# HoangChuongNguyen/ibgs

Hardware: AMD Instinct MI355X
Metric: train-step fps (fwd+bwd raster) @1080p, 1M Gaussians (higher is better)
Workload: dtype f32

## Files before the change

ibgs_amd/csrc/binning.hip:

```cpp
#include "common.h"
#include "wave_bits.h"

namespace ibgs {

constexpr int CB = BIN_CELL;
constexpr int XCHUNK = BIN_XCHUNK;

struct RectU { uint32_t x0, x1, y0, y1; };
struct Footprint { RectU r; uint64_t m0, m1, m2, m3; bool masked, rows; };
static_assert(IBGS_CULL_WORDS == 4, "four mask words");
__device__ __forceinline__ Footprint make_footprint(const uint4 rr, const uint64_t* __restrict__ tmask_hi, uint32_t id)
{
    Footprint f;
    f.r = RectU{rr.x & 0xFFFFu, rr.x >> 16, rr.y & 0xFFFFu, rr.y >> 16};
    const uint32_t area = (f.r.x1 - f.r.x0) * (f.r.y1 - f.r.y0);
    f.masked = area <= (uint32_t)IBGS_CULL_MAX_TILES;
    f.m0 = ((uint64_t)rr.w << 32) | rr.z;
    f.rows = !f.masked && f.m0 == 0ull;
    const uint64_t* mw = tmask_hi + (size_t)id * (IBGS_CULL_WORDS - 1);
    f.m1 = (f.masked && area > 64u) ? mw[0] : 0ull;
    f.m2 = (f.masked && area > 128u) ? mw[1] : 0ull;
    f.m3 = (f.masked && area > 192u) ? mw[2] : 0ull;
    return f;
}
// ... 464 lines not shown
            s_base[c] += (uint32_t)(__popcll(s_touch[c]) + __popcll(s_touch[nc + c]) + __popcll(s_touch[2 * nc + c]) + __popcll(s_touch[3 * nc + c]));
        __syncthreads();
    }
}

__device__ __forceinline__ int cell_of_chunk(const uint32_t* __restrict__ cell_chunk0, int ncells, uint32_t ch)
{
    int lo = 0, hi = ncells;
    while (hi - lo > 1) { const int mid = (lo + hi) >> 1; if (cell_chunk0[mid] <= ch) lo = mid; else hi = mid; }
    return lo;
}

__global__ void __launch_bounds__(64) expand_count_kernel(const uint32_t* __restrict__ cell_start, const uint32_t* __restrict__ cell_chunk0, int ncells,
                                                          const uint4* __restrict__ cent,
                                                          uint32_t* __restrict__ chunk_cnt )
{
    const uint32_t ch = blockIdx.x;
    if (ch >= cell_chunk0[ncells]) return;
    const int lane = threadIdx.x;
    const int cell = cell_of_chunk(cell_chunk0, ncells, ch);
    const uint32_t i0 = cell_start[cell] + (ch - cell_chunk0[cell]) * XCHUNK, i1 = min(cell_start[cell + 1], i0 + XCHUNK);
    uint32_t mlo[XCHUNK / 64], mhi[XCHUNK / 64];
#pragma unroll
    for (int rd = 0; rd < XCHUNK / 64; rd++) {
        const uint32_t i = i0 + (uint32_t)rd * 64 + lane;
        const uint4 e = (i < i1) ? cent[i] : make_uint4(0u, 0u, 0u, 0u);
        mlo[rd] = e.z; mhi[rd] = e.w;
    }
    const BitTransposeConsts btc = bit_transpose_consts(lane);
    uint32_t cnt = 0;
#pragma unroll
    for (int rd = 0; rd < XCHUNK / 64; rd++) {
        if (i0 + (uint32_t)rd * 64 >= i1) break;
        wave_bit_transpose64(mlo[rd], mhi[rd], btc);
        cnt += (uint32_t)__popc(mlo[rd]) + (uint32_t)__popc(mhi[rd]);
    }
    chunk_cnt[(size_t)ch * 64 + lane] = cnt;
}

constexpr int TR_WAVES = 16;
__global__ void __launch_bounds__(64 * TR_WAVES) tile_ranges_kernel(int ntiles, uint32_t* __restrict__ tile_start ,
                                                                   uint32_t* __restrict__ ranges, uint32_t* __restrict__ counters , uint32_t cap,
                                                                   const uint32_t* __restrict__ sort_flag ,
                                                                   uint32_t* __restrict__ host_note , uint32_t note_ticket)
{
    constexpr int NW = TR_WAVES;
    __shared__ uint32_t s_wave[NW];
    const int tid = threadIdx.x, lane = tid & 63, wave = tid >> 6;
    const int per_wave = ((ntiles + NW - 1) / NW + 63) / 64 * 64;
    const int w0 = min(ntiles, wave * per_wave), w1 = min(ntiles, w0 + per_wave);
    constexpr int KEEP = 32;
    const int nsteps = (w1 - w0 + 63) / 64;
    uint32_t v[KEEP];
    uint32_t sum = 0;
#pragma unroll
    for (int k = 0; k < KEEP; k++) { const int t = w0 + k * 64 + lane; v[k] = (k < nsteps && t < w1) ? tile_start[t] : 0u; sum += v[k]; }
    for (int k = KEEP; k < nsteps; k++) { const int t = w0 + k * 64 + lane; sum += t < w1 ? tile_start[t] : 0u; }
#pragma unroll
    for (int d = 32; d >= 1; d >>= 1) sum += (uint32_t)__shfl_xor((int)sum, d, 64);
    if (lane == 0) s_wave[wave] = sum;
    __syncthreads();
    uint32_t run = 0;
    for (int w = 0; w < wave; w++) run += s_wave[w];
    auto step = [&](int k, uint32_t n) {
        uint32_t inc = n;
#pragma unroll
        for (int d = 1; d < 64; d <<= 1) { const uint32_t o = (uint32_t)__shfl_up((int)inc, d, 64); if (lane >= d) inc += o; }
        const uint32_t start = run + inc - n;
        const int t = w0 + k * 64 + lane;
        if (t < w1) {
            tile_start[t] = start;
            const uint32_t a = min(start, cap), b = min(start + n, cap);
            *reinterpret_cast<uint2*>(ranges + 2 * (size_t)t) = (b > a) ? make_uint2(a, b) : make_uint2(0u, 0u);
        }
        run += (uint32_t)__shfl((int)inc, 63, 64);
    };
#pragma unroll
    for (int k = 0; k < KEEP; k++) if (k < nsteps) step(k, v[k]);
    for (int k = KEEP; k < nsteps; k++) { const int t = w0 + k * 64 + lane; step(k, t < w1 ? tile_start[t] : 0u); }
    if (tid == NW * 64 - 1) {
        tile_start[ntiles] = run; counters[0] = run;
        if (host_note) {
            host_note[0] = run; host_note[2] = counters[2]; if (sort_flag && *sort_flag) host_note[3] = 1u;
            __threadfence_system();
            __hip_atomic_store(host_note + 4, note_ticket, __ATOMIC_RELEASE, __HIP_MEMORY_SCOPE_SYSTEM);
        }
    }
}

constexpr int CSCAN_WAVES = 8;
__global__ void __launch_bounds__(64 * CSCAN_WAVES) cell_scan_kernel(const uint32_t* __restrict__ cell_chunk0, int ncells, int cgx, int gx, int gy,
                                                                     uint32_t* __restrict__ chunk_cnt, uint32_t* __restrict__ tile_total )
{
    __shared__ uint32_t s_sum[CSCAN_WAVES][64];
    const int cell = blockIdx.x, lane = threadIdx.x & 63, wave = threadIdx.x >> 6;
    const uint32_t c0 = cell_chunk0[cell], c1 = cell_chunk0[cell + 1];
    const uint32_t per = (c1 - c0 + CSCAN_WAVES - 1) / CSCAN_WAVES;
    const uint32_t w0 = min(c1, c0 + (uint32_t)wave * per), w1 = min(c1, w0 + per);
    uint32_t sum = 0;
    for (uint32_t ch = w0; ch < w1; ch += 8) {
        uint32_t c[8];
#pragma unroll
        for (int k = 0; k < 8; k++) c[k] = (ch + k < w1) ? chunk_cnt[(size_t)(ch + k) * 64 + lane] : 0u;
#pragma unroll
        for (int k = 0; k < 8; k++) sum += c[k];
    }
    s_sum[wave][lane] = sum;
    __syncthreads();
    uint32_t run = 0, total = 0;
#pragma unroll
    for (int w = 0; w < CSCAN_WAVES; w++) { const uint32_t v = s_sum[w][lane]; if (w < wave) run += v; total += v; }
    for (uint32_t ch = w0; ch < w1; ch += 8) {
        uint32_t c[8];
#pragma unroll
        for (int k = 0; k < 8; k++) c[k] = (ch + k < w1) ? chunk_cnt[(size_t)(ch + k) * 64 + lane] : 0u;
#pragma unroll
        for (int k = 0; k < 8; k++) if (ch + k < w1) { chunk_cnt[(size_t)(ch + k) * 64 + lane] = run; run += c[k]; }
    }
    const int tx = (cell % cgx) * CB + (lane & 7), ty = (cell / cgx) * CB + (lane >> 3);
    if (wave == 0 && tx < gx && ty < gy) tile_total[ty * gx + tx] = total;
}

constexpr int SCAT_STAGE = 4096;
__global__ void __launch_bounds__(64) expand_scatter_kernel(const uint32_t* __restrict__ cell_start, const uint32_t* __restrict__ cell_chunk0, int ncells,
                                                            int cgx, int gx, int gy, const uint4* __restrict__ cent,
                                                            const uint32_t* __restrict__ chunk_pref, const uint32_t* __restrict__ tile_start,
                                                            uint32_t cap, uint32_t* __restrict__ point_list)
{
    __shared__ uint32_t s_id[XCHUNK / 64][64];
    __shared__ uint8_t s_out[SCAT_STAGE];
    const uint32_t ch = blockIdx.x;
    if (ch >= cell_chunk0[ncells]) return;
    const int lane = threadIdx.x;
    const int cell = cell_of_chunk(cell_chunk0, ncells, ch);
    const uint32_t i0 = cell_start[cell] + (ch - cell_chunk0[cell]) * XCHUNK, i1 = min(cell_start[cell + 1], i0 + XCHUNK);
    const int tx = (cell % cgx) * CB + (lane & 7), ty = (cell / cgx) * CB + (lane >> 3);
    const uint32_t slot0 = (tx < gx && ty < gy) ? tile_start[ty * gx + tx] + chunk_pref[(size_t)ch * 64 + lane] : 0u;
    uint32_t mlo[XCHUNK / 64], mhi[XCHUNK / 64];
#pragma unroll
    for (int rd = 0; rd < XCHUNK / 64; rd++) {
        const uint32_t i = i0 + (uint32_t)rd * 64 + lane;
        const uint4 e = (i < i1) ? cent[i] : make_uint4(0u, 0u, 0u, 0u);
        mlo[rd] = e.z; mhi[rd] = e.w;
        s_id[rd][lane] = e.x;
    }
    const BitTransposeConsts btc = bit_transpose_consts(lane);
    uint32_t n = 0;
#pragma unroll
    for (int rd = 0; rd < XCHUNK / 64; rd++) {
        if (i0 + (uint32_t)rd * 64 < i1) wave_bit_transpose64(mlo[rd], mhi[rd], btc);
        n += (uint32_t)__popc(mlo[rd]) + (uint32_t)__popc(mhi[rd]);
    }
    uint32_t inc = n;
#pragma unroll
    for (int d = 1; d < 64; d <<= 1) { const uint32_t o = (uint32_t)__shfl_up((int)inc, d, 64); if (lane >= d) inc += o; }
    const uint32_t total = (uint32_t)__builtin_amdgcn_readlane((int)inc, 63);
    const bool staged = total <= (uint32_t)SCAT_STAGE;
    const uint32_t base = inc - n;
    __syncthreads();
    uint32_t k = staged ? base : slot0;
#pragma unroll
    for (int rd = 0; rd < XCHUNK / 64; rd++) {
#pragma unroll
        for (int half = 0; half < 2; half++) {
            uint32_t bits = half ? mhi[rd] : mlo[rd];
            while (bits != 0u) {
                const int l = __builtin_ctz(bits) + 32 * half;
                bits &= bits - 1u;
// ... 87 lines not shown
```

ibgs_amd/csrc/render_bwd.hip:

```cpp
#include "common.h"
#include <stdlib.h>
#include "wave_reduce.h"
#include <type_traits>

namespace ibgs {

struct BwdParams {
    const uint32_t* ranges; const uint32_t* point_list; const float4* rec;
    Cam cam;
    int ntiles;
    TileMap tmap;
    int n_src; int tex_quant;
    int power_skip;
    const uint32_t* tile_risky;
    const float* ref_to_src; const float4* src_rgba;
    const float* final_T; const uint32_t* n_contrib; const float* sum_w; const uint32_t* low_high;
    const int32_t* valid_idx; const float* valid_w;
    const float* depth_pixels; const float* warped_pixels;
    const float* dL_dcolor; const float* dL_dnormal; const float* dL_ddepth; const float* dL_dwarped;
    float* gacc;
    int tab_slots;
    const uint32_t* slot_c; const uint32_t* meta; float* tab;
    const uint32_t* order;
    int slab_ipt;
// ... 643 lines not shown
                        const float S0 = Q[0] + Q[1];
                        const float t = dx0 * S0;
                        v[0] = fmaf(-8.0f, Q[1], t); v[1] = dy0 * S0;
                        v[4] = fmaf(dx0, fmaf(-16.0f, Q[1], t), 64.0f * Q[1]);
                        v[5] = dy0 * v[0]; v[6] = dy0 * v[1];
                        v[7] = S0;
                    } else {
                        const float qdx = Q[0] * dx0, qdy = Q[0] * dy0;
                        v[0] = qdx; v[1] = qdy; v[4] = qdx * dx0; v[5] = qdx * dy0; v[6] = qdy * dy0; v[7] = Q[0];
                    }
                    v[2] = aX; v[3] = aY;
                    v[8] = vR; v[9] = vG; v[10] = vB; v[11] = vNx; v[12] = vNy; v[13] = vNz; v[14] = vD; v[15] = 0.f;
                    const float tot = wave_transpose_reduce16(v, lane);
                    const uint32_t id = __float_as_uint(q0.w);
                    if (col >= 0) {
                        if (p.slab) p.slab[((size_t)(r0 + k) * (p.slab_ipt ? p.slab_ipt : IPT) + (size_t)sub) * GACC_FLOATS + col] = tot;
                        else atomicAdd(p.gacc + (size_t)id * GACC_FLOATS + col, tot);
                    }
                }
            }
        };
        if (bg0) { if (stable) chunk(std::true_type{}, std::true_type{}); else chunk(std::false_type{}, std::true_type{}); }
        else { if (stable) chunk(std::true_type{}, std::false_type{}); else chunk(std::false_type{}, std::false_type{}); }
        __syncthreads();
        top -= count;
    }
}

#ifdef IBGS_TRACE_WAVES
__device__ uint4 g_trace_bwd[IBGS_TRACE_MAX];
#endif
__global__ void __launch_bounds__(64, 8) render_bwd_color_kernel(BwdParams p)
{
    IBGS_TRACE_BEGIN();
    int tile, sub = 0;
    bool have;
    if (p.order) { const uint32_t t = p.order[blockIdx.x]; tile = (int)(t & ~ORDER_SPLIT_BIT); have = t != 0xFFFFFFFFu; }
    else have = tile_map_item(p.tmap, blockIdx.x, p.cam.gx, p.cam.gy, 1, tile, sub);
    __shared__ float4 s_rec[3][BWD_CHUNK];
    __shared__ __align__(16) unsigned char s_pix[4 * WAVE * sizeof(float4)];
    if (have && !tile_is_risky(p.tile_risky, tile)) render_bwd_color_body<4, true, false, true>(p, tile, sub, s_rec, reinterpret_cast<float4 (*)[WAVE]>(s_pix));
    IBGS_TRACE_END(g_trace_bwd);
}
__global__ void __launch_bounds__(64, 8) render_bwd_color_noabs_kernel(BwdParams p)
{
    int tile, sub = 0;
    bool have;
    if (p.order) { const uint32_t t = p.order[blockIdx.x]; tile = (int)(t & ~ORDER_SPLIT_BIT); have = t != 0xFFFFFFFFu; }
    else have = tile_map_item(p.tmap, blockIdx.x, p.cam.gx, p.cam.gy, 1, tile, sub);
    __shared__ float4 s_rec[3][BWD_CHUNK];
    __shared__ __align__(16) unsigned char s_pix[4 * WAVE * sizeof(float4)];
    if (have && !tile_is_risky(p.tile_risky, tile)) render_bwd_color_body<4, false, false, true>(p, tile, sub, s_rec, reinterpret_cast<float4 (*)[WAVE]>(s_pix));
}
template <bool ABS>
__global__ void __launch_bounds__(64, 4) render_bwd_color_risk_kernel(BwdParams p)
{
    __shared__ float4 s_rec[3][BWD_CHUNK];
    __shared__ float4 s_gpix[4][WAVE];
    int tile = (int)blockIdx.x;
    if (p.order) { const uint32_t t = p.order[blockIdx.x]; if (t == 0xFFFFFFFFu) return; tile = (int)(t & ~ORDER_SPLIT_BIT); }
    if (tile >= p.ntiles || !tile_is_risky(p.tile_risky, tile)) return;
    render_bwd_color_body<4, ABS, true>(p, tile, 0, s_rec, s_gpix);
}

constexpr int ORDER_SNAKE_ROUNDS = 8;
__global__ void __launch_bounds__(1024) tile_order_kernel(int ntiles, int nslots , int slot_rounds ,
                                                          const uint32_t* __restrict__ walked_waves, const uint32_t* __restrict__ meta, uint32_t* __restrict__ order,
                                                          uint32_t* __restrict__ order_out ,
                                                          int theta_pct = 0 )
{
    __shared__ uint32_t s_hist[1024];
    __shared__ uint32_t s_w[16];
    __shared__ uint32_t s_max;
    __shared__ unsigned long long s_total;
    const int tid = threadIdx.x, lane = tid & 63, wave = tid >> 6;
    const uint32_t ipt = meta[10];
    if (ipt != 1u && ipt != 2u && ipt != 4u) {
        for (int i = tid; i < nslots; i += 1024) { const uint32_t v = i < ntiles ? ((uint32_t)i | (theta_pct > 0 ? ORDER_SPLIT_BIT : 0u)) : 0xFFFFFFFFu; order[i] = v; if (order_out) order_out[i] = v; }
        return;
    }
    auto walked_of = [&](int t) { uint32_t v = walked_waves[(size_t)t * ipt]; for (uint32_t k = 1; k < ipt; k++) v = max(v, walked_waves[(size_t)t * ipt + k]); return v; };
    s_hist[tid] = 0u;
    if (tid == 0) { s_max = 0u; s_total = 0ull; }
    for (int i = tid; i < nslots; i += 1024) { order[i] = 0xFFFFFFFFu; if (order_out) order_out[i] = 0xFFFFFFFFu; }
    __syncthreads();
    constexpr int KEEP = 16;
    uint32_t w[KEEP];
    uint32_t m = 0;
    unsigned long long sum = 0ull;
#pragma unroll
    for (int k = 0; k < KEEP; k++) { const int t = tid + k * 1024; w[k] = t < ntiles ? walked_of(t) : 0u; m = max(m, w[k]); sum += w[k]; }
    for (int t = tid + KEEP * 1024; t < ntiles; t += 1024) { const uint32_t v = walked_of(t); m = max(m, v); sum += v; }
    for (int d = 32; d >= 1; d >>= 1) m = max(m, (uint32_t)__shfl_xor((int)m, d, 64));
    if (lane == 0) atomicMax(&s_max, m);
    if (theta_pct > 0) {
        for (int d = 32; d >= 1; d >>= 1) sum += __shfl_xor(sum, d, 64);
        if (lane == 0) atomicAdd(&s_total, sum);
    }
    __syncthreads();
    const uint32_t mx = s_max;
    const unsigned long long total = s_total;
    const int sh = mx >= 1024u ? (32 - __builtin_clz(mx)) - 10 : 0;
    auto bucket = [&](uint32_t v) { return 1023u - min(v >> sh, 1023u); };
#pragma unroll
    for (int k = 0; k < KEEP; k++) if (tid + k * 1024 < ntiles) atomicAdd(&s_hist[bucket(w[k])], 1u);
    for (int t = tid + KEEP * 1024; t < ntiles; t += 1024) atomicAdd(&s_hist[bucket(walked_of(t))], 1u);
    __syncthreads();
    const uint32_t v = s_hist[tid];
    uint32_t inc = v;
    for (int d = 1; d < 64; d <<= 1) { const uint32_t o = (uint32_t)__shfl_up((int)inc, d, 64); if (lane >= d) inc += o; }
    if (lane == 63) s_w[wave] = inc;
    __syncthreads();
    uint32_t before = 0;
    for (int ww = 0; ww < wave; ww++) before += s_w[ww];
    s_hist[tid] = before + inc - v;
    __syncthreads();
    const uint32_t nrounds = (uint32_t)nslots / (uint32_t)ORDER_CLASSES;
    auto put = [&](int t, uint32_t key) {
        const uint32_t r = atomicAdd(&s_hist[bucket(key)], 1u);
        const uint32_t stratum = r / ORDER_CLASSES, c = r % ORDER_CLASSES;
        uint32_t slot = r;
        if (nrounds <= (uint32_t)slot_rounds) {
            const uint32_t round = (stratum + 1u) % nrounds;
            slot = round * ORDER_CLASSES + ((stratum & 1u) ? ORDER_CLASSES - 1u - c : c);
        }
        const uint32_t word = (uint32_t)t | ((theta_pct > 0 && hybrid_split(key, total, (uint32_t)theta_pct)) ? ORDER_SPLIT_BIT : 0u);
        order[slot] = word;
        if (order_out) order_out[slot] = word;
    };
#pragma unroll
    for (int k = 0; k < KEEP; k++) if (tid + k * 1024 < ntiles) put(tid + k * 1024, w[k]);
    for (int t = tid + KEEP * 1024; t < ntiles; t += 1024) put(t, walked_of(t));
}
__global__ void __launch_bounds__(64, 8) render_bwd_color_small_kernel(BwdParams p)
{
    int tile, sub;
    __shared__ float4 s_rec[3][BWD_CHUNK];
    __shared__ float4 s_gpix[1][WAVE];
    if (tile_map_item(p.tmap, blockIdx.x, p.cam.gx, p.cam.gy, 4, tile, sub) && !tile_is_risky(p.tile_risky, tile)) render_bwd_color_body<1>(p, tile, sub, s_rec, s_gpix);
}
template <bool ABS>
__global__ void __launch_bounds__(64, 8) render_bwd_color_hybrid_kernel(BwdParams p)
{
    __shared__ float4 s_rec[3][BWD_CHUNK];
    __shared__ float4 s_gpix[4][WAVE];
    int tile, sub; bool split;
    if (!hybrid_item(blockIdx.x, p.hybrid_grid1, p.order, tile, sub, split) || tile_is_risky(p.tile_risky, tile)) return;
    if (split) render_bwd_color_body<1, ABS>(p, tile, sub, s_rec, s_gpix);
    else if (sub == 0) render_bwd_color_body<4, ABS>(p, tile, 0, s_rec, s_gpix);
}
template <int PPL, bool ABS>
__device__ __forceinline__ void render_bwd_geo_entry(const BwdParams& p)
{
    __shared__ float4 s_rec[4][BWD_CHUNK];
    __shared__ float4 s_gpix[PPL][WAVE];
    __shared__ float4 s_gnrm[PPL][WAVE];
    int tile, sub;
    if (PPL == 4 && p.order) { const uint32_t t = p.order[blockIdx.x]; if (t == 0xFFFFFFFFu) return; tile = (int)(t & ~ORDER_SPLIT_BIT); sub = 0; }
    else if (!tile_map_item(p.tmap, blockIdx.x, p.cam.gx, p.cam.gy, 4 / PPL, tile, sub)) return;
    if (tile_is_risky(p.tile_risky, tile)) return;
    render_bwd_geo_body<PPL, ABS>(p, tile, sub, s_rec, s_gpix, s_gnrm);
}
template <bool ABS>
__global__ void __launch_bounds__(64, 3) render_bwd_geo_risk_kernel(BwdParams p)
{
    __shared__ float4 s_rec[4][BWD_CHUNK];
    __shared__ float4 s_gpix[4][WAVE];
    __shared__ float4 s_gnrm[4][WAVE];
    int tile = (int)blockIdx.x;
    if (p.order) { const uint32_t t = p.order[blockIdx.x]; if (t == 0xFFFFFFFFu) return; tile = (int)(t & ~ORDER_SPLIT_BIT); }
    if (tile >= p.ntiles || !tile_is_risky(p.tile_risky, tile)) return;
    render_bwd_geo_body<4, ABS, true>(p, tile, 0, s_rec, s_gpix, s_gnrm);
}
__global__ void __launch_bounds__(64, 4) render_bwd_geo4_kernel(BwdParams p) { render_bwd_geo_entry<4, true>(p); }
__global__ void __launch_bounds__(64, 4) render_bwd_geo4_noabs_kernel(BwdParams p) { render_bwd_geo_entry<4, false>(p); }
__global__ void __launch_bounds__(64, 6) render_bwd_geo_kernel(BwdParams p) { render_bwd_geo_entry<1, true>(p); }
template <bool ABS>
__global__ void __launch_bounds__(64, 4) render_bwd_geo_hybrid_kernel(BwdParams p)
{
    __shared__ float4 s_rec[4][BWD_CHUNK];
    __shared__ float4 s_gpix[4][WAVE];
    __shared__ float4 s_gnrm[4][WAVE];
    int tile, sub; bool split;
    if (!hybrid_item(blockIdx.x, p.hybrid_grid1, p.order, tile, sub, split) || tile_is_risky(p.tile_risky, tile)) return;
    if (split) render_bwd_geo_body<1, ABS>(p, tile, sub, s_rec, s_gpix, s_gnrm);
    else if (sub == 0) render_bwd_geo_body<4, ABS>(p, tile, 0, s_rec, s_gpix, s_gnrm);
}

int render_backward_ref_arith(uint32_t flags)
{
    if (flags & IBGS_FLAG_NO_REF_POWER_SKIP) return 0;
    return RA_DECIDE | ((flags & IBGS_FLAG_REF_ARITH) ? RA_ASSOC : RA_LFORM);
}

int render_backward_waves_per_tile(const ibgs_backward_args& a)
{
    const int nt = ((a.W + TILE - 1) / TILE) * ((a.H + TILE - 1) / TILE);
    if (a.render_geo) return ((a.flags & IBGS_FLAG_QUADRANT_WAVES) ? false : ((a.flags & IBGS_FLAG_TILE_WAVES) ? true : nt >= 4096)) ? 1 : 4;
    return ((a.flags & IBGS_FLAG_QUADRANT_WAVES) ? true : ((a.flags & IBGS_FLAG_TILE_WAVES) ? false : nt < hybrid_max_tiles())) ? 4 : 1;
}

int launch_render_backward(hipStream_t s, const ibgs_backward_args& a, const GeomState& g, const BinState& b,
                           const ImgState& im, const float4* src_rgba, float* slab, float* geo_tab)
{
    BwdParams p;
    p.ranges = im.ranges; p.point_list = b.point_list; p.rec = reinterpret_cast<const float4*>(g.rec);
    p.cam = make_cam(a.viewmatrix, a.projmatrix, a.campos, a.bg, a.tanfovx, a.tanfovy, a.W, a.H);
    p.ntiles = p.cam.gx * p.cam.gy;
// ... 105 lines not shown
```

ibgs_amd/csrc/render_fwd.hip:

```cpp
#include "common.h"

namespace ibgs {

struct FwdParams {
    const uint32_t* ranges; const uint32_t* point_list; const float4* rec;
    Cam cam;
    int ntiles;
    TileMap tmap;
    int n_views, gyv; float fxv[IBGS_MAX_VIEWS], fyv[IBGS_MAX_VIEWS];
    int n_src; int L; float thr; int tex_quant;
    int power_skip;
    const float* ref_to_src; const float* src_cam_pos; const float4* src_rgba; const float* src_depths;
    int ds0, ds1, ds2, ds3, ds4;
    float* final_T; uint32_t* n_contrib; float* sum_w; uint32_t* low_high; int32_t* valid_idx; float* valid_w; uint32_t* slot_c; uint32_t* meta; uint32_t* walked;
    uint32_t* risky;
    int hybrid_grid1;
    int hybrid;
    const uint32_t* order;
    float* out_color; float* out_normal; float* out_depth; float* out_cam_feat; float* out_warped;
    float* out_min_depth_diff; float* out_camera_ray; int32_t* out_mask;
};

enum { MODE_COLOR = 0, MODE_GEO = 1, MODE_DEPTH = 2 };

// ... 86 lines not shown
#pragma unroll
    for (int q = 0; q < PPL; q++) {
        const int qq = quad0 + q;
        px[q] = tx0 + (qq & 1) * 8 + (lane & 7);
        py[q] = ty0 + (qq >> 1) * 8 + (lane >> 3);
        pxf[q] = (float)px[q]; pyf[q] = (float)py[q];
        inside[q] = px[q] < W && py[q] < H;
        live[q] = __builtin_amdgcn_ballot_w64(inside[q]);
        recm[q] = live[q];
        T[q] = 1.0f; C[q][0] = C[q][1] = C[q][2] = 0.f; lastc[q] = 0;
    }
    const float pxf_t0 = (float)(tx0 + (lane & 7)), pyf_t0 = (float)(ty0 + (lane >> 3));
    const float fx = (DEPTH && p.n_views > 1) ? p.fxv[view] : p.cam.fx, fy = (DEPTH && p.n_views > 1) ? p.fyv[view] : p.cam.fy;
    const float cx = (float)(W * 0.5f), cy = (float)(H * 0.5f);
    const float eps = 1.0e-8f;

    float Nacc[PPL][3];
    constexpr bool RING_LDS = GEO && PPL <= 2;
    __shared__ float s_bw[RING_LDS ? PPL : 1][RING_LDS ? MAXL : 1][RING_LDS ? WAVE : 1];
    __shared__ uint32_t s_bc[RING_LDS ? PPL : 1][RING_LDS ? MAXL : 1][RING_LDS ? WAVE : 1];
    float bd[PPL][RING_LDS ? 1 : MAXL], bw[PPL][RING_LDS ? 1 : MAXL]; uint32_t bc[PPL][RING_LDS ? 1 : MAXL];
    int before_ptr[PPL], below_count[PPL];
    float tot_w[PPL], wd_sum[PPL];
    int resume[PPL]; uint32_t cnt[PPL];
    float rayx[PPL], rayy[PPL];
    const int L = p.L;
    if (GEO && blockIdx.x == 0 && lane == 0) p.meta[0] = (uint32_t)L;
    const int before_cap = (L % 2 == 0) ? (L / 2) : ((L + 1) / 2);
    const int below_cap = L - before_cap;
    if (GEO || DEPTH) {
#pragma unroll
        for (int q = 0; q < PPL; q++) {
            Nacc[q][0] = Nacc[q][1] = Nacc[q][2] = 0.f;
#pragma unroll
            for (int s = 0; s < MAXL; s++) {
                if (RING_LDS) { s_bw[q][s][lane] = 0.f; s_bc[q][s][lane] = 0u; }
                else if (s < (RING_LDS ? 1 : MAXL)) { bd[q][s] = 0.f; bw[q][s] = 0.f; bc[q][s] = 0u; }
            }
            before_ptr[q] = 0; below_count[q] = 0; tot_w[q] = 0.f; wd_sum[q] = 0.f; resume[q] = 0; cnt[q] = 0;
            rayx[q] = (pxf[q] - cx) / fx; rayy[q] = (pyf[q] - cy) / fy;
        }
    }

    const uint32_t r0 = p.ranges[2 * tile], r1 = p.ranges[2 * tile + 1];
    const int n = (int)(r1 - r0);

    auto fetch_quad = [&](int base) -> float4 {
        const int e = base + (lane >> 2);
        if (e < n) return p.rec[(size_t)p.point_list[r0 + e] * 4 + (lane & 3)];
        return make_float4(0.f, 0.f, 0.f, 0.f);
    };
    float4 ahead = make_float4(0.f, 0.f, 0.f, 0.f);
    if constexpr (GEO) ahead = fetch_quad(0);
    int base = 0;
    uint64_t riskany = 0ull;
    for (; base < n; base += CHUNK) {
        uint64_t riskm = 0ull;
        if constexpr (GEO) {
            float4 v = ahead;
            const int qd = lane & 3;
            const bool risky = qd == 1 && base + (lane >> 2) < n && conic_takes_ref_power(v.x, v.y, v.z);
            if (qd == 0) v.z = -__builtin_amdgcn_logf(v.z);
            if (qd == 1) { v.x *= EXP2_SCALE; v.y *= EXP2_SCALE; v.z *= EXP2_SCALE; }
            s_rec[qd][lane >> 2] = v;
            if (p.power_skip) riskm = __builtin_amdgcn_ballot_w64(risky);
            ahead = fetch_quad(base + CHUNK);
        } else {
            const int e = base + lane;
            bool risky = false;
            if (e < n) {
                const uint32_t id = p.point_list[r0 + e];
                const float4* r = p.rec + (size_t)id * 4;
                float4 c0 = r[0], c1 = r[1];
                risky = conic_takes_ref_power(c1.x, c1.y, c1.z);
                stage_for_exp2(c0, c1);
                s_rec[0][lane] = c0;
                s_rec[1][lane] = c1;
                s_rec[2][lane] = DEPTH ? r[3] : r[2];
            }
            if (p.power_skip) riskm = __builtin_amdgcn_ballot_w64(risky);
        }
        riskany |= riskm;
        __syncthreads();
        const int count = min(CHUNK, n - base);
        for (int j = 0; j < count; j++) {
            const float4 q0 = s_rec[0][j];
            const float4 q1 = s_rec[1][j];
            const float4 q2 = s_rec[2][j];
            float4 q3 = q2;
            if constexpr (GEO) q3 = s_rec[3][j];
            const int e = base + j;
            IBGS_LANES_ADD(0, 1);
#ifdef IBGS_COUNT_LANES
            bool lc_any_ = false;
#endif
            uint32_t e1v = (uint32_t)(e + 1);
            asm volatile("" : "+v"(e1v));
            const float dx0 = q0.x - (TILE_Q >= 0 ? pxf_t0 : pxf[0]), dy0 = q0.y - (TILE_Q >= 0 ? pyf_t0 : pyf[0]);
            const float lx0 = q1.x * dx0 + q1.y * dy0, ly0 = q1.y * dx0 + q1.z * dy0;
            const float P0 = fmaf(dx0, lx0, fmaf(dy0, ly0, q0.z));
            float p2q[PPL];
            p2q[0] = P0;
            if (PPL >= 2) p2q[1] = fmaf(-16.0f, lx0, P0 + 64.0f * q1.x);
            if (PPL == 4) {
                p2q[2] = fmaf(-16.0f, ly0, P0 + 64.0f * q1.z);
                p2q[3] = fmaf(128.0f, q1.y, p2q[2] + (p2q[1] - P0));
            }
            if constexpr (TILE_Q >= 1 && PPL == 1) {
                const float E1 = fmaf(-16.0f, lx0, P0 + 64.0f * q1.x);
                const float E2 = fmaf(-16.0f, ly0, P0 + 64.0f * q1.z);
                p2q[0] = TILE_Q == 1 ? E1 : (TILE_Q == 2 ? E2 : fmaf(128.0f, q1.y, E2 + (E1 - P0)));
            }
            if ((riskm >> (GEO ? 4 * j + 1 : j)) & 1ull) {
                const uint32_t gid = p.point_list[r0 + e];
                const float4 g0 = p.rec[(size_t)gid * 4], g1 = p.rec[(size_t)gid * 4 + 1];
#pragma unroll
                for (int q = 0; q < PPL; q++) p2q[q] = ref_power_E(g0.x - pxf[q], g0.y - pyf[q], g1.x, g1.y, g1.z, q0.z);
            }
#pragma unroll
            for (int q = 0; q < PPL; q++) {
                if (live[q] == 0ull) continue;
                const float p2 = p2q[q];
                uint64_t m = __builtin_amdgcn_ballot_w64(p2 <= ALPHA_SKIP_E) & live[q];
                if (DEPTH) {
                    const uint64_t running = __builtin_amdgcn_ballot_w64(e >= resume[q]) & live[q];
                    if (__builtin_amdgcn_inverse_ballot_w64(running)) cnt[q]++;
                    m &= running;
                }
                if (m == 0ull) continue;
                IBGS_LANES_ADD(2, 64); IBGS_LANES_ADD(3, __builtin_popcountll(m));
#ifdef IBGS_COUNT_LANES
                lc_any_ = true;
#endif
                const float alpha = fminf(0.99f, __builtin_amdgcn_exp2f(-p2));
                const float aeff = __builtin_amdgcn_inverse_ballot_w64(m) ? alpha : 0.f;
                float aT = aeff * T[q];
                float test_T = T[q] - aT;
                const uint64_t fin = __builtin_amdgcn_ballot_w64(test_T < 0.0001f) & m;
                if (fin != 0ull) {
                    const bool pf = __builtin_amdgcn_inverse_ballot_w64(fin);
                    aT = pf ? 0.f : aT;
                    test_T = pf ? T[q] : test_T;
                    live[q] &= ~fin;
                    m &= ~fin;
                }
                const bool acc = __builtin_amdgcn_inverse_ballot_w64(m);
                const uint32_t contributor = DEPTH ? cnt[q] : e1v;
                if (!DEPTH) { C[q][0] += q2.x * aT; C[q][1] += q2.y * aT; C[q][2] += q2.z * aT; }
                if (GEO) { Nacc[q][0] += q3.x * aT; Nacc[q][1] += q3.y * aT; Nacc[q][2] += q3.z * aT; }
                if ((GEO && (m & recm[q]) != 0ull) || DEPTH) {
                    const float denom = q3.x * rayx[q] + q3.y * rayy[q] + q3.z + eps;
                    float dep = 0.f;
                    if (DEPTH) dep = -q1.w / denom;
                    const bool pos = DEPTH ? (dep > 0.0f) : (q1.w * denom < 0.0f);
                    const bool hit = acc && pos;
                    const bool front = T[q] > 0.5f;
                    int slot = -1;
                    if (hit && front) slot = before_ptr[q];
                    else if (hit && below_count[q] < below_cap) slot = before_cap + below_count[q];
                    if (DEPTH && slot >= 0 && front) {
                        float oldw = 0.f, oldd = 0.f;
#pragma unroll
                        for (int s = 0; s < (RING_LDS ? 1 : MAXL); s++) if (s == slot) { oldw = bw[q][s]; oldd = bd[q][s]; }
                        tot_w[q] -= oldw; wd_sum[q] -= oldw * oldd;
                    }
                    if (slot >= 0) {
                        if (RING_LDS) { s_bw[q][slot][lane] = aT; s_bc[q][slot][lane] = contributor; }
                        else {
#pragma unroll
                            for (int s = 0; s < (RING_LDS ? 1 : MAXL); s++) if (s == slot) { if (DEPTH) bd[q][s] = dep; bw[q][s] = aT; bc[q][s] = contributor; }
                        }
                        if (front) { const int nb = before_ptr[q] + 1; before_ptr[q] = (nb == before_cap) ? 0 : nb; }
                        else below_count[q]++;
                        if (DEPTH) { tot_w[q] += aT; wd_sum[q] += aT * dep; }
                    }
                    if (DEPTH && hit && below_count[q] == below_cap) {
                        resume[q] = (e / 256 + 1) * 256;
                    }
                    if (DEPTH && below_cap > 0) {
                        live[q] &= ~__builtin_amdgcn_ballot_w64(hit && below_count[q] == below_cap);
                    }
                    if (GEO) recm[q] &= ~__builtin_amdgcn_ballot_w64(test_T <= 0.5f && below_count[q] >= below_cap);
                }
                T[q] = test_T;
                lastc[q] = acc ? contributor : lastc[q];
            }
#ifdef IBGS_COUNT_LANES
            if (lc_any_) IBGS_LANES_ADD(1, 1);
#endif
        }
        __syncthreads();
        uint64_t anylive = 0ull;
#pragma unroll
        for (int q = 0; q < PPL; q++) anylive |= live[q];
        if (anylive == 0ull) break;
    }

#pragma unroll
    for (int q = 0; q < PPL; q++) {
        if (!inside[q]) continue;
        const size_t pix = vbase + (size_t)py[q] * W + px[q];
        p.final_T[pix] = T[q];
        p.n_contrib[pix] = lastc[q];
        if (!DEPTH) {
            p.out_color[pix] = C[q][0] + T[q] * p.cam.bg[0];
            p.out_color[HW + pix] = C[q][1] + T[q] * p.cam.bg[1];
            p.out_color[2 * HW + pix] = C[q][2] + T[q] * p.cam.bg[2];
        }
        if (DEPTH) p.out_depth[pix] = wd_sum[q] / (tot_w[q] + eps);
        if (GEO) { p.out_normal[pix] = Nacc[q][0]; p.out_normal[HW + pix] = Nacc[q][1]; p.out_normal[2 * HW + pix] = Nacc[q][2]; }
    }
    {
        uint32_t m = 0;
#pragma unroll
        for (int q = 0; q < PPL; q++) m = max(m, inside[q] ? lastc[q] : 0u);
#pragma unroll
        for (int d = 32; d >= 1; d >>= 1) m = max(m, (uint32_t)__shfl_xor((int)m, d, WAVE));
        if (p.hybrid) {
            if (IPT == 1) { if (lane < 4) p.walked[(size_t)tile * 4 + lane] = lane == 0 ? m : 0u; }
            else if (lane == 0) p.walked[(size_t)tile * 4 + sub] = m;
            if (lane == 0 && tile == 0 && sub == 0) p.meta[10] = 4u;
        }
        else if (lane == 0) { p.walked[(size_t)tile * IPT + sub] = m; if (tile == 0 && sub == 0) p.meta[10] = (uint32_t)IPT; }
        if (!DEPTH && p.risky && lane < PPL) p.risky[(size_t)tile * 4 + sub + lane * IPT] = riskany != 0ull ? 1u : 0u;
    }
    if (GEO) {
#pragma clang fp contract(off)
#pragma unroll 1
        for (int q = 0; q < PPL; q++) {
            const int qq = quad0 + q;
            const int pxq = tx0 + (qq & 1) * 8 + (lane & 7), pyq = ty0 + (qq >> 1) * 8 + (lane >> 3);
            if (!(pxq < W && pyq < H)) continue;
            const size_t pix = vbase + (size_t)pyq * W + pxq;
            const float pxfq = (float)pxq, pyfq = (float)pyq;
            const float rayxq = (pxfq - cx) / fx, rayyq = (pyfq - cy) / fy;
            const float inv_fx = 1.0f / fx, inv_fy = 1.0f / fy;
            const float pdx = pxfq - cx, pdy = pyfq - cy;
            float dv[RING_LDS ? 1 : MAXL];
            float tw = 0.f, med = 0.f;
            uint32_t lo = RING_LDS ? s_bc[q][0][lane] : bc[q][0], hi = lo;
#pragma unroll 1
            for (int s = 0; s < L; s++) {
                float w = 0.f; uint32_t c = 0;
                if (RING_LDS) { w = s_bw[q][s][lane]; c = s_bc[q][s][lane]; }
                else {
#pragma unroll
                    for (int k = 0; k < (RING_LDS ? 1 : MAXL); k++) if (k == s) { w = bw[q][k]; c = bc[q][k]; }
                }
                p.slot_c[(size_t)s * HW + pix] = (w == 0.0f) ? 0u : c;
                float d = 0.f;
                if (w != 0.0f) {
                    const uint32_t gid = p.point_list[r0 + c - 1u];
                    const float4 g1 = p.rec[(size_t)gid * 4 + 1], g3 = p.rec[(size_t)gid * 4 + 3];
                    d = -g1.w / (g3.x * rayxq + g3.y * rayyq + g3.z + eps);
                    tw += w; med += w * d;
                    lo = min(lo, c); hi = max(hi, c);
                }
                if (RING_LDS) s_bc[q][s][lane] = __float_as_uint(d);
                else {
#pragma unroll
                    for (int k = 0; k < (RING_LDS ? 1 : MAXL); k++) if (k == s) dv[k] = d;
                }
            }
// ... 214 lines not shown
```

ibgs_amd/csrc/scan_sort.hip:

```cpp
#include "common.h"
#include "sh_color.h"
#include <cstdlib>

namespace ibgs {

constexpr int SCAN_THREADS = 256;
constexpr int SCAN_ITEMS = 8;
constexpr int SCAN_CHUNK = SCAN_THREADS * SCAN_ITEMS;

constexpr int RS_THREADS = 256;
constexpr int RS_ITEMS = 16;
constexpr int RS_CHUNK = RS_THREADS * RS_ITEMS;
constexpr int RS_MAX_BINS = 256;

__device__ __forceinline__ uint32_t wave_inclusive_scan(uint32_t v, int lane)
{
#pragma unroll
    for (int d = 1; d < WAVE; d <<= 1) {
        const uint32_t o = __shfl_up(v, d, WAVE);
        if (lane >= d) v += o;
    }
    return v;
}

// ... 208 lines not shown
    }
    __syncthreads();
#pragma unroll
    for (int k = 0; k < RS_ITEMS; k++) {
        const uint32_t l = (uint32_t)k * RS_THREADS + threadIdx.x;
        if (l < count) {
            const uint32_t kk = skey[l];
            const uint32_t d = (kk >> shift) & mask;
            const uint32_t dst = l + delta[d];
            keys_out[dst] = (K)kk;
            vals_out[dst] = sval[l];
        }
    }
}


constexpr uint32_t OS_FLAG_AGG = 1u << 30, OS_FLAG_INC = 2u << 30, OS_VAL_MASK = (1u << 30) - 1u;
constexpr int OS_MAX_PASS = 4;
constexpr int OS_HIST_THREADS = 1024;
constexpr int OS_THREADS = 512, OS_WAVES = OS_THREADS / 64, OS_ITEMS = RS_CHUNK / OS_THREADS;

template <int NT>
__device__ __forceinline__ void onesweep_hist_block(const uint32_t* __restrict__ keys, size_t n, int npass, int dbits, uint32_t* __restrict__ ghist,
                                                    int drop_max, uint32_t* __restrict__ n_kept, unsigned nblk, uint32_t (*h)[RS_MAX_BINS], uint32_t* s_kept)
{
    for (int k = threadIdx.x; k < OS_MAX_PASS * RS_MAX_BINS; k += NT) (&h[0][0])[k] = 0;
    if (threadIdx.x == 0) *s_kept = 0;
    __syncthreads();
    const uint32_t mask = (1u << dbits) - 1u;
    const size_t stride = (size_t)nblk * NT;
    uint32_t kept = 0;
    for (size_t i = (size_t)blockIdx.x * NT + threadIdx.x; i < n; i += stride) {
        const uint32_t k = keys[i];
        if (drop_max && k == 0xFFFFFFFFu) continue;
        kept++;
        for (int p = 0; p < npass; p++) atomicAdd(&h[p][(k >> (p * dbits)) & mask], 1u);
    }
    if (kept) atomicAdd(s_kept, kept);
    __syncthreads();
    if (threadIdx.x == 0 && *s_kept) atomicAdd(n_kept, *s_kept);
    for (int k = threadIdx.x; k < npass * RS_MAX_BINS; k += NT) {
        const uint32_t c = (&h[0][0])[k];
        if (c) atomicAdd(&ghist[k], c);
    }
}

__global__ void __launch_bounds__(OS_HIST_THREADS) onesweep_hist_kernel(const uint32_t* __restrict__ keys, size_t n, int npass, int dbits,
                                                                   uint32_t* __restrict__ ghist ,
                                                                   int drop_max , uint32_t* __restrict__ n_kept)
{
    __shared__ uint32_t h[OS_MAX_PASS][RS_MAX_BINS];
    __shared__ uint32_t s_kept;
    onesweep_hist_block<OS_HIST_THREADS>(keys, n, npass, dbits, ghist, drop_max, n_kept, gridDim.x, h, &s_kept);
}

struct OsPassLds {
    unsigned long long ptab[OS_WAVES][RS_MAX_BINS];
    uint32_t wcnt[OS_WAVES][RS_MAX_BINS];
    uint32_t dstart[RS_MAX_BINS];
    uint32_t delta[RS_MAX_BINS];
    uint32_t lds_wave[4];
    uint32_t skey[RS_CHUNK];
    uint32_t sval[RS_CHUNK];
    uint32_t s_bid;
};

__device__ __forceinline__ void onesweep_pass_block(const uint32_t* __restrict__ keys_in, const uint32_t* __restrict__ vals_in,
                                                   uint32_t* __restrict__ keys_out, uint32_t* __restrict__ vals_out,
                                                   size_t n, int shift, int nbits, int nbins,
                                                   const uint32_t* __restrict__ ghist ,
                                                   uint32_t* __restrict__ status ,
                                                   uint32_t* __restrict__ ticket, uint32_t* __restrict__ err,
                                                   int drop_here ,
                                                   const uint32_t* __restrict__ n_kept ,
                                                   uint32_t* __restrict__ stays ,
                                                   uint32_t spin_limit ,
                                                   OsPassLds& L)
{
    auto& wcnt = L.wcnt; auto& ptab = L.ptab; auto& dstart = L.dstart; auto& delta = L.delta; auto& lds_wave = L.lds_wave; auto& skey = L.skey; auto& sval = L.sval; auto& s_bid = L.s_bid;

    const int lane = threadIdx.x & 63, wave = threadIdx.x >> 6;
    const uint32_t kept = *n_kept;
    const size_t n_in = drop_here ? n : (size_t)kept;
    if (threadIdx.x == 0) s_bid = atomicAdd(ticket, 1u);
    for (int k = threadIdx.x; k < OS_WAVES * RS_MAX_BINS; k += OS_THREADS) { (&wcnt[0][0])[k] = 0; (&ptab[0][0])[k] = 0ull; }
    __syncthreads();
    const uint32_t bid = s_bid;
    const size_t base = (size_t)bid * RS_CHUNK;
    if (base >= n_in) return;

    const int all_one_bin = __syncthreads_or((int)(threadIdx.x < (unsigned)nbins && kept != 0u && ghist[threadIdx.x] == kept));
    if (all_one_bin && (!drop_here || (size_t)kept == n)) {
        if (stays) { if (bid == 0 && threadIdx.x == 0) *stays = 1u; return; }
#pragma unroll
        for (int k = 0; k < OS_ITEMS; k++) {
            const size_t idx = base + (size_t)k * OS_THREADS + threadIdx.x;
            if (idx < n_in) { keys_out[idx] = keys_in[idx]; vals_out[idx] = vals_in[idx]; }
        }
        return;
    }

    const uint32_t mask = (uint32_t)nbins - 1;
    const uint64_t lt_mask = (lane == 0) ? 0ull : (~0ull >> (64 - lane));

    uint32_t key[OS_ITEMS], val[OS_ITEMS], rank[OS_ITEMS];
    uint32_t takes = 0;
#pragma unroll
    for (int k = 0; k < OS_ITEMS; k++) {
        const size_t idx = base + (size_t)wave * (OS_ITEMS * 64) + (size_t)k * 64 + lane;
        const bool inside = idx < n_in;
        key[k] = inside ? keys_in[idx] : 0xFFFFFFFFu;
        val[k] = inside ? vals_in[idx] : 0u;
        const bool valid = inside && !(drop_here && key[k] == 0xFFFFFFFFu);
        takes |= valid ? (1u << k) : 0u;
        const uint32_t d = (key[k] >> shift) & mask;
        const uint32_t r = wave_rank(d, valid, lane, lt_mask, &wcnt[wave][0], &ptab[wave][0]);
        rank[k] = r;
    }
    __syncthreads();

    uint32_t tot = 0;
    if (threadIdx.x < nbins) {
#pragma unroll
        for (int w = 0; w < OS_WAVES; w++) { const uint32_t c = wcnt[w][threadIdx.x]; wcnt[w][threadIdx.x] = tot; tot += c; }
        uint32_t* mine = status + (size_t)bid * RS_MAX_BINS + threadIdx.x;
        __hip_atomic_store(mine, (bid == 0 ? OS_FLAG_INC : OS_FLAG_AGG) | tot, __ATOMIC_RELAXED, __HIP_MEMORY_SCOPE_AGENT);
    }
    uint32_t gtotal, ltotal;
    const uint32_t gstart = block_exclusive_scan_256(threadIdx.x < nbins ? ghist[threadIdx.x] : 0u, &gtotal, lds_wave);
    const uint32_t ds = block_exclusive_scan_256(tot, &ltotal, lds_wave);
    if (spin_limit == 0u && bid == 0 && threadIdx.x == 0) *err = 1u;
    if (threadIdx.x < nbins) {
        uint32_t excl = 0;
        if (bid > 0) {
            constexpr int LOOKBACK = 8;
            int64_t b = (int64_t)bid - 1;
            uint32_t spins = 0;
            bool done = false;
            while (!done && b >= 0) {
                uint32_t st[LOOKBACK];
#pragma unroll
                for (int k = 0; k < LOOKBACK; k++)
                    st[k] = (b - k >= 0) ? __hip_atomic_load(status + (size_t)(b - k) * RS_MAX_BINS + threadIdx.x, __ATOMIC_RELAXED, __HIP_MEMORY_SCOPE_AGENT)
                                         : OS_FLAG_INC;
                int used = 0;
#pragma unroll
                for (int k = 0; k < LOOKBACK; k++) {
                    if (done || used != k) continue;
                    const uint32_t flag = st[k] & ~OS_VAL_MASK;
                    if (flag == 0u) continue;
                    excl += st[k] & OS_VAL_MASK;
                    used = k + 1;
                    if (flag == OS_FLAG_INC) done = true;
                }
                b -= used;
                if (!done && used < LOOKBACK) {
                    if (++spins > (spin_limit ? spin_limit : (1u << 26))) { *err = 1u; break; }
                    __builtin_amdgcn_s_sleep(1);
                }
            }
            __hip_atomic_store(status + (size_t)bid * RS_MAX_BINS + threadIdx.x, OS_FLAG_INC | ((excl + tot) & OS_VAL_MASK),
                               __ATOMIC_RELAXED, __HIP_MEMORY_SCOPE_AGENT);
        }
        dstart[threadIdx.x] = ds;
        delta[threadIdx.x] = gstart + excl - ds;
    }
    __syncthreads();

    const uint32_t count = ltotal;
#pragma unroll
    for (int k = 0; k < OS_ITEMS; k++) {
        if (takes & (1u << k)) {
            const uint32_t d = (key[k] >> shift) & mask;
            const uint32_t lpos = dstart[d] + wcnt[wave][d] + rank[k];
            skey[lpos] = key[k];
            sval[lpos] = val[k];
// ... 248 lines not shown
```

Measured before the change: 626.1.

## Trim fences, early-exit finished waves, vectorize tile-order loads, early one-bin sort exit

Bundles several unrelated micro-optimizations. The host-note publish replaces a system-wide fence with a release fence, a waitcnt and a relaxed store. tile_order now loads walked counts as vectors specialised by ipt and only fills the empty tail slots instead of clearing the whole order array first. The forward rasterizer stops its gaussian loop once no pixel in the wave is live, and the onesweep pass returns before the ticket atomic and LDS clearing when all keys fall into one bin. The weakened fence could break host visibility ordering, and the tail fill relies on slot_of mapping ranks to every unused slot.

After: 629.7 (median of 3 runs). No clear change (+0.6%).

```diff
diff --git a/ibgs_amd/csrc/binning.hip b/ibgs_amd/csrc/binning.hip
--- a/ibgs_amd/csrc/binning.hip
+++ b/ibgs_amd/csrc/binning.hip
@@ -570,8 +570,9 @@
         tile_start[ntiles] = run; counters[0] = run;
         if (host_note) {
             host_note[0] = run; host_note[2] = counters[2]; if (sort_flag && *sort_flag) host_note[3] = 1u;
-            __threadfence_system();
-            __hip_atomic_store(host_note + 4, note_ticket, __ATOMIC_RELEASE, __HIP_MEMORY_SCOPE_SYSTEM);
+            __builtin_amdgcn_fence(__ATOMIC_RELEASE, "");
+            asm volatile("s_waitcnt vmcnt(0)" ::: "memory");
+            __hip_atomic_store(host_note + 4, note_ticket, __ATOMIC_RELAXED, __HIP_MEMORY_SCOPE_SYSTEM);
         }
     }
 }
diff --git a/ibgs_amd/csrc/render_bwd.hip b/ibgs_amd/csrc/render_bwd.hip
--- a/ibgs_amd/csrc/render_bwd.hip
+++ b/ibgs_amd/csrc/render_bwd.hip
@@ -749,14 +749,24 @@
     auto walked_of = [&](int t) { uint32_t v = walked_waves[(size_t)t * ipt]; for (uint32_t k = 1; k < ipt; k++) v = max(v, walked_waves[(size_t)t * ipt + k]); return v; };
     s_hist[tid] = 0u;
     if (tid == 0) { s_max = 0u; s_total = 0ull; }
-    for (int i = tid; i < nslots; i += 1024) { order[i] = 0xFFFFFFFFu; if (order_out) order_out[i] = 0xFFFFFFFFu; }
     __syncthreads();
     constexpr int KEEP = 16;
     uint32_t w[KEEP];
     uint32_t m = 0;
     unsigned long long sum = 0ull;
-#pragma unroll
-    for (int k = 0; k < KEEP; k++) { const int t = tid + k * 1024; w[k] = t < ntiles ? walked_of(t) : 0u; m = max(m, w[k]); sum += w[k]; }
+    auto load_kept = [&](auto ipt_tag) {
+        constexpr int IPT = decltype(ipt_tag)::value;
+#pragma unroll
+        for (int k = 0; k < KEEP; k++) {
+            const uint32_t* wp = walked_waves + (size_t)min(tid + k * 1024, ntiles - 1) * IPT;
+            if constexpr (IPT == 1) w[k] = wp[0];
+            else if constexpr (IPT == 2) { const uint2 v = *reinterpret_cast<const uint2*>(wp); w[k] = max(v.x, v.y); }
+            else { const uint4 v = *reinterpret_cast<const uint4*>(wp); w[k] = max(max(v.x, v.y), max(v.z, v.w)); }
+        }
+    };
+    if (ipt == 1u) load_kept(std::integral_constant<int, 1>{}); else if (ipt == 2u) load_kept(std::integral_constant<int, 2>{}); else load_kept(std::integral_constant<int, 4>{});
+#pragma unroll
+    for (int k = 0; k < KEEP; k++) { w[k] = tid + k * 1024 < ntiles ? w[k] : 0u; m = max(m, w[k]); sum += w[k]; }
     for (int t = tid + KEEP * 1024; t < ntiles; t += 1024) { const uint32_t v = walked_of(t); m = max(m, v); sum += v; }
     for (int d = 32; d >= 1; d >>= 1) m = max(m, (uint32_t)__shfl_xor((int)m, d, 64));
     if (lane == 0) atomicMax(&s_max, m);
@@ -783,14 +793,18 @@
     s_hist[tid] = before + inc - v;
     __syncthreads();
     const uint32_t nrounds = (uint32_t)nslots / (uint32_t)ORDER_CLASSES;
-    auto put = [&](int t, uint32_t key) {
-        const uint32_t r = atomicAdd(&s_hist[bucket(key)], 1u);
+    auto slot_of = [&](uint32_t r) {
         const uint32_t stratum = r / ORDER_CLASSES, c = r % ORDER_CLASSES;
         uint32_t slot = r;
         if (nrounds <= (uint32_t)slot_rounds) {
             const uint32_t round = (stratum + 1u) % nrounds;
             slot = round * ORDER_CLASSES + ((stratum & 1u) ? ORDER_CLASSES - 1u - c : c);
         }
+        return slot;
+    };
+    for (uint32_t r = (uint32_t)ntiles + (uint32_t)tid; r < (uint32_t)nslots; r += 1024u) { const uint32_t slot = slot_of(r); order[slot] = 0xFFFFFFFFu; if (order_out) order_out[slot] = 0xFFFFFFFFu; }
+    auto put = [&](int t, uint32_t key) {
+        const uint32_t slot = slot_of(atomicAdd(&s_hist[bucket(key)], 1u));
         const uint32_t word = (uint32_t)t | ((theta_pct > 0 && hybrid_split(key, total, (uint32_t)theta_pct)) ? ORDER_SPLIT_BIT : 0u);
         order[slot] = word;
         if (order_out) order_out[slot] = word;
diff --git a/ibgs_amd/csrc/render_fwd.hip b/ibgs_amd/csrc/render_fwd.hip
--- a/ibgs_amd/csrc/render_fwd.hip
+++ b/ibgs_amd/csrc/render_fwd.hip
@@ -192,7 +192,13 @@
         }
         riskany |= riskm;
         __syncthreads();
-        const int count = min(CHUNK, n - base);
+        int count = min(CHUNK, n - base);
+        auto leave_if_finished = [&]() {
+            uint64_t anyl = 0ull;
+#pragma unroll
+            for (int q = 0; q < PPL; q++) anyl |= live[q];
+            if (anyl == 0ull) count = 0;
+        };
         for (int j = 0; j < count; j++) {
             const float4 q0 = s_rec[0][j];
             const float4 q1 = s_rec[1][j];
@@ -253,6 +259,7 @@
                     test_T = pf ? T[q] : test_T;
                     live[q] &= ~fin;
                     m &= ~fin;
+                    leave_if_finished();
                 }
                 const bool acc = __builtin_amdgcn_inverse_ballot_w64(m);
                 const uint32_t contributor = DEPTH ? cnt[q] : e1v;
@@ -288,7 +295,8 @@
                         resume[q] = (e / 256 + 1) * 256;
                     }
                     if (DEPTH && below_cap > 0) {
-                        live[q] &= ~__builtin_amdgcn_ballot_w64(hit && below_count[q] == below_cap);
+                        const uint64_t full = __builtin_amdgcn_ballot_w64(hit && below_count[q] == below_cap);
+                        if (full != 0ull) { live[q] &= ~full; leave_if_finished(); }
                     }
                     if (GEO) recm[q] &= ~__builtin_amdgcn_ballot_w64(test_T <= 0.5f && below_count[q] >= below_cap);
                 }
diff --git a/ibgs_amd/csrc/scan_sort.hip b/ibgs_amd/csrc/scan_sort.hip
--- a/ibgs_amd/csrc/scan_sort.hip
+++ b/ibgs_amd/csrc/scan_sort.hip
@@ -314,6 +314,10 @@
     const int lane = threadIdx.x & 63, wave = threadIdx.x >> 6;
     const uint32_t kept = *n_kept;
     const size_t n_in = drop_here ? n : (size_t)kept;
+    if (stays) {
+        const int one_bin = __syncthreads_or((int)(threadIdx.x < (unsigned)nbins && kept != 0u && ghist[threadIdx.x] == kept));
+        if (one_bin && (!drop_here || (size_t)kept == n)) { if (blockIdx.x == 0 && threadIdx.x == 0) *stays = 1u; return; }
+    }
     if (threadIdx.x == 0) s_bid = atomicAdd(ticket, 1u);
     for (int k = threadIdx.x; k < OS_WAVES * RS_MAX_BINS; k += OS_THREADS) { (&wcnt[0][0])[k] = 0; (&ptab[0][0])[k] = 0ull; }
     __syncthreads();
@@ -323,7 +327,6 @@
 
     const int all_one_bin = __syncthreads_or((int)(threadIdx.x < (unsigned)nbins && kept != 0u && ghist[threadIdx.x] == kept));
     if (all_one_bin && (!drop_here || (size_t)kept == n)) {
-        if (stays) { if (bid == 0 && threadIdx.x == 0) *stays = 1u; return; }
 #pragma unroll
         for (int k = 0; k < OS_ITEMS; k++) {
             const size_t idx = base + (size_t)k * OS_THREADS + threadIdx.x;
```
